# solislemuslab/BayesianNetworkRegression.jl

Measured on NVIDIA B200. Metric: gibbs_iters_per_sec_all_chains, higher is better.
Workload: dtype f64

## Files before the change

bayesiannetworkregression.jl_b200/csrc/bnr_linalg.cu:

```cuda
#include <cstdio>
#include <cstdlib>
#include <cstring>
#include <cuda.h>
#include "bnr_engine.cuh"
#include "bnr_kernels.h"

namespace bnr {

__device__ __forceinline__ void dmma884(double& c0, double& c1, double a, double b) {
  asm volatile("mma.sync.aligned.m8n8k4.row.col.f64.f64.f64.f64 {%0,%1}, {%2}, {%3}, {%0,%1};\n"
               : "+d"(c0), "+d"(c1) : "d"(a), "d"(b));
}
__device__ __forceinline__ double neg_bits(double x) {
  return __longlong_as_double(__double_as_longlong(x) ^ (long long)0x8000000000000000ull);
}
__device__ __forceinline__ void cp_async_commit() { asm volatile("cp.async.commit_group;\n" ::); }
template <int N>
__device__ __forceinline__ void cp_async_wait() { asm volatile("cp.async.wait_group %0;\n" ::"n"(N)); }
__device__ __forceinline__ void cp_async16(void* smem, const void* gmem) {
  const unsigned sa = (unsigned)__cvta_generic_to_shared(smem);
  asm volatile("cp.async.cg.shared.global [%0], [%1], 16;\n" ::"r"(sa), "l"(gmem));
}

__device__ __forceinline__ unsigned smem_u32(const void* p) { return (unsigned)__cvta_generic_to_shared(p); }
// ... 1191 lines not shown
#pragma unroll
        for (int h = 0; h < BW_NH; ++h)
#pragma unroll
          for (int q = 0; q < BW_CPW; ++q) bJ[h * BW_COLS + warp * BW_CPW + q] = xn[h][q];
      }
      __syncwarp();
      named_bar_sync(1, 256);
    }
    for (int id = tid; id < nown * PB; id += 256) {
      const int I = r + BWC_K * (id / PB);
      if (I < T) out[(size_t)c * out_stride + (size_t)I * PB + id % PB] = xo[id];
    }
  }
  cluster_sync_all();
}

__global__ void k_copy_sym(const double* __restrict__ G, size_t chain_stride, int np, double* __restrict__ out) {
  const int c = blockIdx.y, j = blockIdx.x;
  const double* Gc = G + (size_t)c * chain_stride;
  double* o = out + (size_t)c * np * np;
  for (int i = threadIdx.x; i < np; i += blockDim.x) {
    const double v = (i >= j) ? Gc[(size_t)j * np + i] : Gc[(size_t)i * np + j];
    o[(size_t)j * np + i] = v;
  }
}

constexpr int XM_BM = 128, XM_BN = 64, XM_BK = 16, XM_STAGES = 3;
constexpr int XM_LDM = 132, XM_LDK = 20;
constexpr int XM_A_DBL = (XM_BK * XM_LDM > XM_BM * XM_LDK) ? XM_BK * XM_LDM : XM_BM * XM_LDK;
constexpr int XM_STAGE_DBL = XM_A_DBL + XM_BN * XM_LDK;
constexpr size_t XMMA_SMEM = sizeof(double) * XM_STAGES * XM_STAGE_DBL;

__device__ __forceinline__ void cp_async16_zfill(void* smem, const void* gmem, bool valid) {
  const unsigned sa = (unsigned)__cvta_generic_to_shared(smem);
  const int sz = valid ? 16 : 0;
  asm volatile("cp.async.cg.shared.global [%0], [%1], 16, %2;\n" ::"r"(sa), "l"(gmem), "r"(sz));
}

template <int TRANS>
__global__ void __launch_bounds__(256) k_xmma(const double* __restrict__ X, int np, int M, int K, int N,
                                              const double* __restrict__ in, int ldin, double* __restrict__ out,
                                              int ldout, int k_per_split) {
  extern __shared__ __align__(16) double sm[];
  const int tid = threadIdx.x, lane = tid & 31, warp = tid >> 5;
  const int lk = lane & 3, lr = lane >> 2, wm = warp & 3, wn = warp >> 2;
  const int m0 = blockIdx.x * XM_BM, n0 = blockIdx.y * XM_BN;
  const int kbeg = blockIdx.z * k_per_split;
  const int kend = min(K, kbeg + k_per_split);
  const int nsteps = (kend - kbeg + XM_BK - 1) / XM_BK;
  double* o = out + (size_t)blockIdx.z * N * ldout;

  auto load_stage = [&](int step) {
    double* As = sm + (size_t)(step % XM_STAGES) * XM_STAGE_DBL;
    double* Vs = As + XM_A_DBL;
    const int k0 = kbeg + step * XM_BK;
    if (TRANS == 0) {
#pragma unroll
      for (int r = 0; r < 4; ++r) {
        const int id = tid + 256 * r, kk = id >> 6, mm = (id & 63) * 2;
        cp_async16_zfill(As + kk * XM_LDM + mm, X + (size_t)(k0 + kk) * np + m0 + mm, m0 + mm < M);
      }
    } else {
#pragma unroll
      for (int r = 0; r < 4; ++r) {
        const int id = tid + 256 * r, mm = id >> 3, kk = (id & 7) * 2;
        const bool ok = m0 + mm < M;
        cp_async16_zfill(As + mm * XM_LDK + kk, X + (size_t)(ok ? m0 + mm : 0) * np + k0 + kk, ok);
      }
    }
#pragma unroll
    for (int r = 0; r < 2; ++r) {
      const int id = tid + 256 * r, nn = id >> 3, kk = (id & 7) * 2;
      const bool ok = n0 + nn < N;
      cp_async16_zfill(Vs + nn * XM_LDK + kk, in + (size_t)(ok ? n0 + nn : 0) * ldin + k0 + kk, ok);
    }
  };

  double acc[4][4][2];
#pragma unroll
  for (int a = 0; a < 4; ++a)
#pragma unroll
    for (int b = 0; b < 4; ++b) acc[a][b][0] = acc[a][b][1] = 0.0;
  int nfv = (N - n0 - wn * 32 + 7) >> 3;
  nfv = nfv < 0 ? 0 : (nfv > 4 ? 4 : nfv);

  for (int s = 0; s < XM_STAGES - 1; ++s) {
    if (s < nsteps) load_stage(s);
    cp_async_commit();
  }
  for (int step = 0; step < nsteps; ++step) {
    cp_async_wait<XM_STAGES - 2>();
    __syncthreads();
    if (step + XM_STAGES - 1 < nsteps) load_stage(step + XM_STAGES - 1);
    cp_async_commit();
    const double* As = sm + (size_t)(step % XM_STAGES) * XM_STAGE_DBL;
    const double* Vs = As + XM_A_DBL;
    if (nfv == 0) continue;
#pragma unroll
    for (int k4 = 0; k4 < XM_BK / 4; ++k4) {
      const int kr = k4 * 4 + lk;
      double af[4], bf[4];
#pragma unroll
      for (int mf = 0; mf < 4; ++mf)
        af[mf] = (TRANS == 0) ? As[kr * XM_LDM + wm * 32 + mf * 8 + lr] : As[(wm * 32 + mf * 8 + lr) * XM_LDK + kr];
#pragma unroll
      for (int nf = 0; nf < 4; ++nf) bf[nf] = (nf < nfv) ? Vs[(wn * 32 + nf * 8 + lr) * XM_LDK + kr] : 0.0;
#pragma unroll
      for (int nf = 0; nf < 4; ++nf) {
        if (nf < nfv) {
#pragma unroll
          for (int mf = 0; mf < 4; ++mf) dmma884(acc[mf][nf][0], acc[mf][nf][1], af[mf], bf[nf]);
        }
      }
    }
  }
  cp_async_wait<0>();
#pragma unroll
  for (int mf = 0; mf < 4; ++mf) {
    const int mm = m0 + wm * 32 + mf * 8 + lr;
#pragma unroll
    for (int nf = 0; nf < 4; ++nf) {
      const int nn = n0 + wn * 32 + nf * 8 + 2 * lk;
      if (mm < M) {
        if (nn < N) o[(size_t)nn * ldout + mm] = acc[mf][nf][0];
        if (nn + 1 < N) o[(size_t)(nn + 1) * ldout + mm] = acc[mf][nf][1];
      }
    }
  }
}

__global__ void k_splitk_reduce(const double* __restrict__ ws, double* __restrict__ out, size_t count, int splits) {
  const size_t i = (size_t)blockIdx.x * blockDim.x + threadIdx.x;
  if (i >= count) return;
  double s = 0.0;
  for (int z = 0; z < splits; ++z) s += ws[(size_t)z * count + i];
  out[i] = s;
}

static int x_times_splits(const Dims& d, int trans) {
  const int M = trans ? d.qp : d.np, K = trans ? d.np : d.qp;
  const int tiles = ((M + XM_BM - 1) / XM_BM) * ((d.C_total + XM_BN - 1) / XM_BN);
  int ks = (2 * 148 + tiles - 1) / tiles;
  const int kmax = K / (4 * XM_BK) > 0 ? K / (4 * XM_BK) : 1;
  if (ks > kmax) ks = kmax;
  if (ks > 64) ks = 64;
  if (ks < 1) ks = 1;
  return ks;
}

size_t x_times_workspace_doubles(const Dims& d) {
  const int a = x_times_splits(d, 0), b = x_times_splits(d, 1);
  const size_t wa = (size_t)a * d.C_total * d.np, wb = (size_t)b * d.C_total * d.qp;
  return wa > wb ? wa : wb;
}

void launch_x_times(const Engine& e, int trans, const double* in, double* out, double* ws, cudaStream_t s) {
  const Dims& d = e.d;
  const int M = trans ? d.qp : d.np, K = trans ? d.np : d.qp, N = d.C;
  const int ldin = trans ? d.np : d.qp, ldout = trans ? d.qp : d.np;
  const int ks = x_times_splits(d, trans);
  const int kper = ((K + ks - 1) / ks + XM_BK - 1) / XM_BK * XM_BK;
  dim3 grid((M + XM_BM - 1) / XM_BM, (N + XM_BN - 1) / XM_BN, ks);
  double* dst = ks == 1 ? out : ws;
  ++g_launches;
  if (trans) k_xmma<1><<<grid, 256, XMMA_SMEM, s>>>(e.X, d.np, M, K, N, in, ldin, dst, ldout, kper);
  else k_xmma<0><<<grid, 256, XMMA_SMEM, s>>>(e.X, d.np, M, K, N, in, ldin, dst, ldout, kper);
  if (ks > 1) {
    const size_t count = (size_t)N * ldout;
    ++g_launches; k_splitk_reduce<<<(unsigned)((count + 255) / 256), 256, 0, s>>>(ws, out, count, ks);
  }
}

__global__ void k_gram_i8(const __grid_constant__ CUtensorMap tmA, const __grid_constant__ CUtensorMap tmB,
                          const double* __restrict__ rscale, double* __restrict__ G, int np, int nvalid, int nkb);
extern const size_t GI_SMEM_BYTES;

void linalg_setup() {
  cudaFuncSetAttribute(k_xmma<0>, cudaFuncAttributeMaxDynamicSharedMemorySize, (int)XMMA_SMEM);
  cudaFuncSetAttribute(k_xmma<1>, cudaFuncAttributeMaxDynamicSharedMemorySize, (int)XMMA_SMEM);
  cudaFuncSetAttribute(k_gram_syrk, cudaFuncAttributeMaxDynamicSharedMemorySize, (int)SYRK_SMEM);
  cudaFuncSetAttribute(k_gram_i8, cudaFuncAttributeMaxDynamicSharedMemorySize, (int)GI_SMEM_BYTES);
  cudaFuncSetAttribute(k_chol_update, cudaFuncAttributeMaxDynamicSharedMemorySize, (int)SYRK_SMEM);
  cudaFuncSetAttribute(k_trsm_dmma, cudaFuncAttributeMaxDynamicSharedMemorySize, (int)SYRK_SMEM);
  cudaFuncSetAttribute(k_potf2_inv, cudaFuncAttributeMaxDynamicSharedMemorySize, (int)POTF2_SMEM);
  cudaFuncSetAttribute(k_bwd_stream, cudaFuncAttributeMaxDynamicSharedMemorySize, 227 * 1024);
  cudaFuncSetAttribute(k_bwd_cluster, cudaFuncAttributeMaxDynamicSharedMemorySize, 227 * 1024);
  cudaFuncSetAttribute(k_small_tile<1, 4>, cudaFuncAttributeMaxDynamicSharedMemorySize, (int)small_tile_smem(32));
  cudaFuncSetAttribute(k_small_tile<2, 4>, cudaFuncAttributeMaxDynamicSharedMemorySize, (int)small_tile_smem(32));
  cudaFuncSetAttribute(k_small_tile<1, 2>, cudaFuncAttributeMaxDynamicSharedMemorySize, (int)small_tile_smem(16));
  cudaFuncSetAttribute(k_small_tile<2, 2>, cudaFuncAttributeMaxDynamicSharedMemorySize, (int)small_tile_smem(16));
  cudaFuncSetAttribute(k_small_tile<1, 8>, cudaFuncAttributeMaxDynamicSharedMemorySize, (int)small_tile_smem(64));
  cudaFuncSetAttribute(k_small_tile<2, 8>, cudaFuncAttributeMaxDynamicSharedMemorySize, (int)small_tile_smem(64));
}

typedef CUresult (*TmapEncodeFn)(CUtensorMap*, CUtensorMapDataType, cuuint32_t, void*, const cuuint64_t*, const cuuint64_t*,
                                 const cuuint32_t*, const cuuint32_t*, CUtensorMapInterleave, CUtensorMapSwizzle,
                                 CUtensorMapL2promotion, CUtensorMapFloatOOBfill);
static TmapEncodeFn g_tmap_encode = nullptr;
bool tmap_setup() {
  if (g_tmap_encode) return true;
  void* fn = nullptr;
  cudaDriverEntryPointQueryResult qr;
  if (cudaGetDriverEntryPoint("cuTensorMapEncodeTiled", &fn, cudaEnableDefault, &qr) != cudaSuccess ||
      qr != cudaDriverEntryPointSuccess || !fn)
    return false;
  g_tmap_encode = (TmapEncodeFn)fn;
  return true;
}
static CUresult encode_map(CUtensorMap* m, const double* base, uint64_t rows, uint64_t krows, uint64_t ld, uint32_t box_rows,
                           uint32_t box_k) {
  memset(m, 0, sizeof(*m));
  const cuuint64_t dims[2] = {rows, krows};
  const cuuint64_t strides[1] = {ld * sizeof(double)};
  const cuuint32_t box[2] = {box_rows, box_k};
  const cuuint32_t estr[2] = {1, 1};
  if (!tmap_setup()) return CUDA_ERROR_NOT_SUPPORTED;
  return g_tmap_encode(m, CU_TENSOR_MAP_DATA_TYPE_FLOAT64, 2, const_cast<double*>(base), dims, strides, box, estr,
                       CU_TENSOR_MAP_INTERLEAVE_NONE, CU_TENSOR_MAP_SWIZZLE_NONE, CU_TENSOR_MAP_L2_PROMOTION_L2_256B,
                       CU_TENSOR_MAP_FLOAT_OOB_FILL_NONE);
}
static CUtensorMap make_map(const double* base, uint64_t rows, uint64_t krows, uint64_t ld, uint32_t box_rows,
                            uint32_t box_k = SY_BK) {
  CUtensorMap m;
  const CUresult r = encode_map(&m, base, rows, krows, ld, box_rows, box_k);
  if (r != CUDA_SUCCESS) {
    fprintf(stderr, "[bnr] cuTensorMapEncodeTiled failed (%d) for a %llu x %llu operand, box %u x %d\n", (int)r,
            (unsigned long long)rows, (unsigned long long)krows, box_rows, (int)box_k);
    abort();
  }
  return m;
}
bool tmaps_check(const Engine& e) {
  const Dims& d = e.d;
  const uint64_t N = d.gdim, C = d.C, T = d.gdim / SY_BT;
  CUtensorMap m;
  bool ok = true;
  if (d.gmode != 2) ok = ok && encode_map(&m, e.X, d.np, d.qp, d.np, SY_LDS, SY_BK) == CUDA_SUCCESS;
  for (uint32_t box : {(uint32_t)SY_LDS, (uint32_t)(SY_BT / 2 + 4), (uint32_t)(SY_BT / 4 + 4)})
    ok = ok && encode_map(&m, e.G, N, N * C, N, box, SY_BK) == CUDA_SUCCESS;
  ok = ok && encode_map(&m, e.Linv, SY_BT, SY_BT * T * C, SY_BT, SY_LDS, SY_BK) == CUDA_SUCCESS;
  ok = ok && encode_map(&m, e.G, N, N * C, N, SY_BT, BW_COLS) == CUDA_SUCCESS;
  ok = ok && encode_map(&m, e.Linv, SY_BT, SY_BT * T * C, SY_BT, SY_BT, BW_COLS) == CUDA_SUCCESS;
  return ok;
}

int syrk_splits(const Dims& d, int C) {
  const int T = d.np / SY_BT, tiles = T * (T + 1) / 2, nk = d.qp / SY_BK;
  if (const char* ov = getenv("BNR_SYRK_SPLITS")) {
    int s = atoi(ov);
    if (s > nk / 8) s = nk / 8;
    return s < 1 ? 1 : (s > SYRK_MAX_SPLITS ? SYRK_MAX_SPLITS : s);
  }
  if (tiles * C >= 148) return 1;
  int s = (4 * 148 + tiles * C - 1) / (tiles * C);
  if (s > nk / 24) s = nk / 24;
  if (s > SYRK_MAX_SPLITS) s = SYRK_MAX_SPLITS;
  return s < 1 ? 1 : s;
}

#ifndef BNR_GI_BK
#define BNR_GI_BK 64
#endif
#ifndef BNR_GI_STAGES
#define BNR_GI_STAGES 2
#endif
constexpr int GI_S = 7;
constexpr int GI_BM = 128, GI_BN = 64;
constexpr int GI_BK = BNR_GI_BK;
constexpr int GI_STAGES = BNR_GI_STAGES;
constexpr int GI_A_PLANE = GI_BM * GI_BK, GI_B_PLANE = GI_BN * GI_BK;
constexpr int GI_STAGE_BYTES = GI_S * (GI_A_PLANE + GI_B_PLANE);
constexpr size_t GI_SMEM = (size_t)GI_STAGES * GI_STAGE_BYTES + 1024 + 256;
const size_t GI_SMEM_BYTES = GI_SMEM;
constexpr int GI_THREADS = 192;
static_assert(GI_BK == 32 || GI_BK == 64 || GI_BK == 128, "k-block = swizzle width");
static_assert(GI_S * GI_BN <= 512, "accumulators exceed tensor memory");

__device__ __forceinline__ unsigned long long gi_desc(unsigned saddr) {
  constexpr unsigned long long layout = GI_BK == 128 ? 2ull : (GI_BK == 64 ? 4ull : 6ull);
  return (unsigned long long)((saddr & 0x3FFFF) >> 4) | (1ull << 16) | ((unsigned long long)((GI_BK * 8) >> 4) << 32) |
         (1ull << 46) | (layout << 61);
}
__host__ __device__ constexpr unsigned gi_idesc(int n) {
  return (2u << 4) | (1u << 7) | (1u << 10) | ((unsigned)(n >> 3) << 17) | ((unsigned)(GI_BM >> 4) << 24);
}

__device__ __forceinline__ void tma_load_3d(void* smem_dst, const CUtensorMap* tm, int x, int y, int z, unsigned long long* bar) {
  asm volatile("cp.async.bulk.tensor.3d.shared::cluster.global.tile.mbarrier::complete_tx::bytes [%0], [%1, {%2, %3, %4}], [%5];\n" ::"r"(
                   smem_u32(smem_dst)), "l"((unsigned long long)tm), "r"(x), "r"(y), "r"(z), "r"(smem_u32(bar)) : "memory");
}
__device__ __forceinline__ void umma_i8(unsigned tmem_d, unsigned long long adesc, unsigned long long bdesc, unsigned idesc,
                                        bool acc) {
  asm volatile("{\n.reg .pred p;\nsetp.ne.b32 p, %4, 0;\ntcgen05.mma.cta_group::1.kind::i8 [%0], %1, %2, %3, p;\n}\n" ::"r"(tmem_d),
               "l"(adesc), "l"(bdesc), "r"(idesc), "r"((int)acc));
}
__device__ __forceinline__ void umma_commit(unsigned long long* bar) {
  asm volatile("tcgen05.commit.cta_group::1.mbarrier::arrive::one.shared::cluster.b64 [%0];\n" ::"r"(smem_u32(bar)) : "memory");
}
__device__ __forceinline__ void tmem_ld8(unsigned taddr, int (&r)[8]) {
  asm volatile("tcgen05.ld.sync.aligned.32x32b.x8.b32 {%0,%1,%2,%3,%4,%5,%6,%7}, [%8];\n"
               : "=r"(r[0]), "=r"(r[1]), "=r"(r[2]), "=r"(r[3]), "=r"(r[4]), "=r"(r[5]), "=r"(r[6]), "=r"(r[7]) : "r"(taddr));
}

__global__ void __launch_bounds__(256) k_gram_slice(const double* __restrict__ X, const double* __restrict__ S, int np,
                                                    int q, int qp, signed char* __restrict__ planes,
                                                    double* __restrict__ rscale) {
  __shared__ unsigned buf[GI_S][32][33];
  __shared__ double red[8][32];
  const int c = blockIdx.y, r0 = blockIdx.x * 32, lane = threadIdx.x & 31, warp = threadIdx.x >> 5;
  const int row = r0 + lane;
  const double* Sc = S + (size_t)c * qp;
  double m = 0.0;
  for (int k0 = warp; k0 < q; k0 += 8 * 32) {
    const int kl = k0 + 8 * lane;
    const double sq = kl < q ? sqrt(Sc[kl]) : 0.0;
    const int nk = (q - k0 + 7) / 8 < 32 ? (q - k0 + 7) / 8 : 32;
    for (int j = 0; j < nk; ++j) m = fmax(m, fabs(X[row + (size_t)np * (k0 + 8 * j)] * __shfl_sync(0xffffffffu, sq, j)));
  }
  red[warp][lane] = m;
  __syncthreads();
  m = 0.0;
#pragma unroll
  for (int w = 0; w < 8; ++w) m = fmax(m, red[w][lane]);
  int p = 0;
  if (m > 0.0) {
    p = 54 - ilogb(m);
    if (ldexp(m, p) > 126.0 * 0x1p48) --p;
  }
  if (warp == 0) rscale[(size_t)c * np + row] = ldexp(1.0, -p);
  const int p1 = p > 1000 ? 1000 : p;
  const double sc1 = ldexp(1.0, p1), sc2 = ldexp(1.0, p - p1);
  signed char* out = planes + (size_t)c * GI_S * np * qp;
  for (int k0 = 0; k0 < qp; k0 += 128) {
    const int kl = k0 + warp * 16 + (lane & 15);
    const double sq = kl < q ? sqrt(Sc[kl]) : 0.0;
#pragma unroll
    for (int g = 0; g < 4; ++g) {
      const int kw = warp * 4 + g;
      unsigned w[GI_S] = {0, 0, 0, 0, 0, 0, 0};
#pragma unroll
      for (int b = 0; b < 4; ++b) {
        const int k = k0 + kw * 4 + b;
        const double sqk = __shfl_sync(0xffffffffu, sq, g * 4 + b);
        if (k < q) {
          const long long M = __double2ll_rn(X[row + (size_t)np * k] * sqk * sc1 * sc2) + 0x808080808080ll;
          const unsigned lo = (unsigned)M ^ 0x80808080u, hi = (unsigned)(M >> 32) ^ 0x8080u;
#pragma unroll
          for (int i = 0; i < 4; ++i) w[GI_S - 1 - i] |= ((lo >> (8 * i)) & 255u) << (8 * b);
#pragma unroll
          for (int i = 0; i < 3; ++i) w[2 - i] |= ((hi >> (8 * i)) & 255u) << (8 * b);
        }
      }
#pragma unroll
      for (int s = 0; s < GI_S; ++s) buf[s][lane][kw] = w[s];
    }
    __syncthreads();
    for (int id = threadIdx.x; id < GI_S * 32 * 32; id += 256) {
      const int s = id >> 10, rr = (id >> 5) & 31, kw = id & 31;
      const int k = k0 + kw * 4;
      if (k < qp) *reinterpret_cast<unsigned*>(out + ((size_t)s * np + r0 + rr) * qp + k) = buf[s][rr][kw];
    }
    __syncthreads();
  }
}

__global__ void __launch_bounds__(GI_THREADS, 1)
k_gram_i8(const __grid_constant__ CUtensorMap tmA, const __grid_constant__ CUtensorMap tmB,
          const double* __restrict__ rscale, double* __restrict__ G, int np, int nvalid, int nkb) {
  extern __shared__ __align__(1024) unsigned char gsm_raw[];
  unsigned char* gsm = reinterpret_cast<unsigned char*>(((size_t)gsm_raw + 1023) & ~(size_t)1023);
  unsigned long long* full = reinterpret_cast<unsigned long long*>(gsm + (size_t)GI_STAGES * GI_STAGE_BYTES);
  unsigned long long* empty = full + GI_STAGES;
  unsigned long long* accf = empty + GI_STAGES;
  unsigned* tmem_slot = reinterpret_cast<unsigned*>(accf + 1);
  const int tid = threadIdx.x, lane = tid & 31, warp = tid >> 5;
  const int c = blockIdx.y;
  int ib = 0;
  while (2 * (ib + 1) * (ib + 2) / 2 <= (int)blockIdx.x) ++ib;
  const int jb = (int)blockIdx.x - ib * (ib + 1);
  const int i0 = ib * GI_BM, j0 = jb * GI_BN;
  const bool diag_block = (j0 / GI_BM) == ib;
  int rows_st = GI_BM;
  if (!diag_block) {
    int nfv = (nvalid - i0 + 7) / 8;
    if (nfv <= 0) return;
    rows_st = (nfv < 4 ? 4 : nfv) * 8;
  }
  if (tid == 0) {
    for (int s = 0; s < GI_STAGES; ++s) { mbar_init(&full[s], 1); mbar_init(&empty[s], 1); }
    mbar_init(accf, 1);
    asm volatile("fence.mbarrier_init.release.cluster;\n" ::: "memory");
  }
  if (warp == 0) {
    asm volatile("tcgen05.alloc.cta_group::1.sync.aligned.shared::cta.b32 [%0], 512;\n" ::"r"(smem_u32(tmem_slot)));
    asm volatile("tcgen05.relinquish_alloc_permit.cta_group::1.sync.aligned;\n");
  }
  asm volatile("tcgen05.fence::before_thread_sync;\n" ::: "memory");
  __syncthreads();
  asm volatile("tcgen05.fence::after_thread_sync;\n" ::: "memory");
  const unsigned tmem = *tmem_slot;

  if (warp == 4 && lane == 0) {
#if defined(GI_LAB_MMA_ONLY)
    for (int kb = 0; kb < GI_STAGES && kb < nkb; ++kb) {
#else
    for (int kb = 0; kb < nkb; ++kb) {
#endif
      const int st = kb % GI_STAGES;
      mbar_wait(&empty[st], ((kb / GI_STAGES) & 1) ^ 1);
      unsigned char* sa = gsm + (size_t)st * GI_STAGE_BYTES;
      mbar_expect_tx(&full[st], GI_STAGE_BYTES);
      tma_load_3d(sa, &tmA, kb * GI_BK, i0, c * GI_S, &full[st]);
      tma_load_3d(sa + GI_S * GI_A_PLANE, &tmB, kb * GI_BK, j0, c * GI_S, &full[st]);
    }
  } else if (warp == 5 && lane == 0) {
    for (int kb = 0; kb < nkb; ++kb) {
      const int st = kb % GI_STAGES;
#if defined(GI_LAB_MMA_ONLY)
      if (kb < GI_STAGES) mbar_wait(&full[st], 0);
#else
      mbar_wait(&full[st], (kb / GI_STAGES) & 1);
#endif
      asm volatile("tcgen05.fence::after_thread_sync;\n" ::: "memory");
#if defined(GI_LAB_LOADS_ONLY)
      umma_commit(&empty[st]);
      continue;
#endif
      const unsigned sa = smem_u32(gsm + (size_t)st * GI_STAGE_BYTES), sb = sa + GI_S * GI_A_PLANE;
#pragma unroll
      for (int kk = 0; kk < GI_BK / 32; ++kk) {
#pragma unroll
        for (int s = 0; s < GI_S; ++s) {
          const unsigned long long ad = gi_desc(sa + s * GI_A_PLANE + kk * 32);
#pragma unroll
          for (int t0 = 0; t0 < GI_S - s; t0 += 4) {
            const int nt = GI_S - s - t0 < 4 ? GI_S - s - t0 : 4;
            umma_i8(tmem + (unsigned)((s + t0) * GI_BN), ad, gi_desc(sb + t0 * GI_B_PLANE + kk * 32), gi_idesc(nt * GI_BN),
                    kb > 0 || kk > 0 || s > 0);
          }
        }
      }
      umma_commit(&empty[st]);
    }
    umma_commit(accf);
  } else if (warp < 4) {
    mbar_wait(accf, 0);
    asm volatile("tcgen05.fence::after_thread_sync;\n" ::: "memory");
    const int r = warp * 32 + lane, i = i0 + r;
    const double ri = rscale[(size_t)c * np + i] * 0x1p96;
    double* Gc = G + (size_t)c * np * np;
    const unsigned trow = tmem + ((unsigned)(warp * 32) << 16);
    for (int j8 = 0; j8 < GI_BN; j8 += 8) {
      int acc[GI_S][8];
#pragma unroll
      for (int g = 0; g < GI_S; ++g) tmem_ld8(trow + (unsigned)(g * GI_BN + j8), acc[g]);
      asm volatile("tcgen05.wait::ld.sync.aligned;\n" ::: "memory");
#pragma unroll
      for (int jj = 0; jj < 8; ++jj) {
        const int j = j0 + j8 + jj;
        double v = (double)acc[GI_S - 1][jj];
#pragma unroll
        for (int g = GI_S - 2; g >= 0; --g) v = (double)acc[g][jj] + v * 0x1p-8;
        v = v * ri * rscale[(size_t)c * np + j];
        if (i == j) v += 1.0;
        if (r < rows_st && (i >> 3) >= (j >> 3)) Gc[(size_t)j * np + i] = v;
      }
    }
  }
  asm volatile("tcgen05.fence::before_thread_sync;\n" ::: "memory");
  __syncthreads();
  if (warp == 0) {
    asm volatile("tcgen05.fence::after_thread_sync;\n" ::: "memory");
    asm volatile("tcgen05.dealloc.cta_group::1.sync.aligned.b32 %0, 512;\n" ::"r"(tmem));
  }
}

bool gram_i8_selected(const Dims& d) { return d.gmode == 1 && d.qp >= GRAM_I8_QP_MIN && d.qp <= GRAM_I8_QP_MAX; }

size_t gram_i8_plane_bytes(const Dims& d) { return (size_t)GI_S * d.np * d.qp; }

static CUresult encode_planes_map(CUtensorMap* m, const signed char* planes, const Dims& d, int C, uint32_t box_rows) {
  memset(m, 0, sizeof(*m));
  const cuuint64_t dims[3] = {(cuuint64_t)d.qp, (cuuint64_t)d.np, (cuuint64_t)GI_S * C};
  const cuuint64_t strides[2] = {(cuuint64_t)d.qp, (cuuint64_t)d.qp * d.np};
  const cuuint32_t box[3] = {(cuuint32_t)GI_BK, box_rows, (cuuint32_t)GI_S};
  const cuuint32_t estr[3] = {1, 1, 1};
  const CUtensorMapSwizzle sw = GI_BK == 128 ? CU_TENSOR_MAP_SWIZZLE_128B
                                             : (GI_BK == 64 ? CU_TENSOR_MAP_SWIZZLE_64B : CU_TENSOR_MAP_SWIZZLE_32B);
  if (!tmap_setup()) return CUDA_ERROR_NOT_SUPPORTED;
  return g_tmap_encode(m, CU_TENSOR_MAP_DATA_TYPE_UINT8, 3, const_cast<signed char*>(planes), dims, strides, box, estr,
                       CU_TENSOR_MAP_INTERLEAVE_NONE, sw, CU_TENSOR_MAP_L2_PROMOTION_L2_256B, CU_TENSOR_MAP_FLOAT_OOB_FILL_NONE);
}

static void launch_gram_i8_products(const Engine& e, cudaStream_t s) {
  const Dims& d = e.d;
  CUtensorMap tmA, tmB;
  if (encode_planes_map(&tmA, e.gram_planes, d, d.C, GI_BM) != CUDA_SUCCESS ||
      encode_planes_map(&tmB, e.gram_planes, d, d.C, GI_BN) != CUDA_SUCCESS) {
    fprintf(stderr, "[bnr] cuTensorMapEncodeTiled failed for the Gram digit planes (%d x %d)\n", d.np, d.qp);
    abort();
  }
  const int T = d.np / GI_BM;
  ++g_launches; k_gram_i8<<<dim3(T * (T + 1), d.C), GI_THREADS, GI_SMEM, s>>>(tmA, tmB, e.gram_rscale, e.G, d.np, d.n,
                                                                             (d.qp + GI_BK - 1) / GI_BK);
}

static void launch_gram_i8(const Engine& e, cudaStream_t s) {
  const Dims& d = e.d;
  ++g_launches; k_gram_slice<<<dim3(d.np / 32, d.C), 256, 0, s>>>(e.X, e.S, d.np, d.q, d.qp, e.gram_planes, e.gram_rscale);
  launch_gram_i8_products(e, s);
}

void launch_syrk_G(const Engine& e, cudaStream_t s) {
  const Dims& d = e.d;
  if (gram_i8_selected(d)) {
    launch_gram_i8(e, s);
    if (e.aux.G_copy) {
      dim3 g2(d.np, d.C);
      ++g_launches; k_copy_sym<<<g2, 256, 0, s>>>(e.G, (size_t)d.np * d.np, d.np, e.aux.G_copy);
    }
    return;
  }
  const int T = d.np / SY_BT;
  const int nk = d.qp / SY_BK;
  const int ns = e.syrk_ws ? e.syrk_ws_cap + 1 : 1;
  const int nk_split = (nk + ns - 1) / ns;
#if defined(SYRK_LAB_ONLY_DIAG)
  dim3 grid(d.C, ns, T);
#elif defined(SYRK_LAB_ONLY_OFFDIAG)
  dim3 grid(d.C, ns, T * (T - 1) / 2);
#else
  dim3 grid(d.C, ns, T * (T + 1) / 2);
#endif
  const size_t gs = (size_t)d.np * d.np;
  const CUtensorMap tmX = make_map(e.X, d.np, d.qp, d.np, SY_LDS);
  ++g_launches; k_gram_syrk<<<grid, SY_THREADS, SYRK_SMEM, s>>>(tmX, e.S, (size_t)d.qp, e.G, gs, d.np, d.n, nk, 1.0,
                                                            nk_split, e.syrk_ws, e.syrk_ws_cap);
  if (ns > 1) {
    dim3 g2(T * (T + 1) / 2 * 8, d.C);
    ++g_launches; k_syrk_splitk_reduce<<<g2, 256, 0, s>>>(e.G, gs, d.np, e.syrk_ws, e.syrk_ws_cap, ns - 1);
  }
  if (e.aux.G_copy) {
    dim3 g2(d.np, d.C);
    ++g_launches; k_copy_sym<<<g2, 256, 0, s>>>(e.G, gs, d.np, e.aux.G_copy);
  }
}

void launch_xtx(const Dims& d, const double* XT, const double* ones, double* XtX, cudaStream_t s) {
  const int T = d.qp / SY_BT;
  dim3 grid(1, 1, T * (T + 1) / 2);
  const CUtensorMap tmXT = make_map(XT, d.qp, d.np, d.qp, SY_LDS);
  ++g_launches; k_gram_syrk<<<grid, SY_THREADS, SYRK_SMEM, s>>>(tmXT, ones, 0, XtX, 0, d.qp, d.q, d.np / SY_BK, 0.0,
                                                            d.np / SY_BK, nullptr, 0);
}

__global__ void __launch_bounds__(256) k_build_P(Engine e) {
  const Dims& d = e.d;
  if (blockIdx.x < blockIdx.y) return;
  const int c = blockIdx.z, N = d.qp;
  const int i = blockIdx.x * 32 + threadIdx.x;
  const double it2 = 1.0 / e.tau2[c];
  double* Gc = e.G + (size_t)c * N * N;
#pragma unroll
  for (int jj = 0; jj < 4; ++jj) {
    const int j = blockIdx.y * 32 + threadIdx.y * 4 + jj;
    if (i < j) continue;
    double v;
    if (i < d.q) {
      v = e.XtX[(size_t)j * N + i] * it2;
      if (i == j) v = (e.XtX[(size_t)j * N + i] + 1.0 / e.S[(size_t)c * d.qp + j]) * it2;
    } else {
      v = (i == j) ? 1.0 : 0.0;
    }
    Gc[(size_t)j * N + i] = v;
  }
}

void launch_build_P(const Engine& e, cudaStream_t s) {
  const Dims& d = e.d;
  dim3 grid(d.qp / 32, d.qp / 32, d.C), block(32, 8);
  ++g_launches; k_build_P<<<grid, block, 0, s>>>(e);
  if (e.aux.G_copy) {
    dim3 g2(d.qp, d.C);
    ++g_launches; k_copy_sym<<<g2, 256, 0, s>>>(e.G, (size_t)d.qp * d.qp, d.qp, e.aux.G_copy);
  }
}

void launch_cholesky(const Engine& e, double* rhs, const ForkJoin& fj, cudaStream_t s) {
  const Dims& d = e.d;
  const int N = d.gdim;
  const int m = d.gmode == 2 ? d.q : d.n;
  const size_t cs = (size_t)N * N;
  const int T = N / PB;
  const size_t ls = (size_t)T * PB * PB;
  static const bool serial = getenv("BNR_CHOL_SERIAL") != nullptr;
  static const int forced = getenv("BNR_CHOL_SCHEDULE") ? atoi(getenv("BNR_CHOL_SCHEDULE")) : 0;
  const bool latency = forced ? forced == 2 : (long long)d.C_total * (T - 1) <= 128;
  ++g_launches; k_augment<<<d.C, 256, 0, s>>>(e.G, cs, N, m, rhs, d.gmode == 2 ? d.qp : d.np, d.gmode == 2 ? e.S : nullptr, e.tau2);
  const CUtensorMap mG = make_map(e.G, N, (uint64_t)N * d.C, N, SY_LDS);
  const CUtensorMap mG2 = make_map(e.G, N, (uint64_t)N * d.C, N, SY_BT / 2 + 4);
  const CUtensorMap mG4 = make_map(e.G, N, (uint64_t)N * d.C, N, SY_BT / 4 + 4);
  const CUtensorMap mL = make_map(e.Linv, PB, (uint64_t)PB * T * d.C, PB, SY_LDS);
  auto mI = [&](int ns) -> const CUtensorMap& { return ns == 4 ? mG4 : (ns == 2 ? mG2 : mG); };

  if (!latency) {
    const bool can_fork = !serial && fj.side != nullptr;
    static const bool a_lo = getenv("BNR_CHOL_A_SIDE_LO") != nullptr;
    cudaStream_t sideA = (!a_lo && fj.side_hi) ? fj.side_hi : fj.side;
    for (int J = 0; J < T; ++J) {
      const bool fork = can_fork && J > 0 && J + 1 < T;
      if (J > 0) {
        const int nk = J * PB / SY_BK;
        if (fork) {
          cudaEventRecord(fj.fork, s);
          cudaStreamWaitEvent(sideA, fj.fork, 0);
          dim3 g2(d.C, T - J - 1);
          ++g_launches; k_chol_update<<<g2, SY_THREADS, SYRK_SMEM, sideA>>>(mG, mG, 0, e.G, cs, N, m + 1, nk, J, J + 1, 1);
          cudaEventRecord(fj.join, sideA);
          dim3 g1(d.C, 1);
          ++g_launches; k_chol_update<<<g1, SY_THREADS, SYRK_SMEM, s>>>(mG, mG, 0, e.G, cs, N, m + 1, nk, J, J, 1);
        } else {
          dim3 g2(d.C, T - J);
          ++g_launches; k_chol_update<<<g2, SY_THREADS, SYRK_SMEM, s>>>(mG, mG, 0, e.G, cs, N, m + 1, nk, J, J, 1);
        }
      }
      ++g_launches; k_potf2_inv<<<d.C, 256, POTF2_SMEM, s>>>(e.G, cs, N, J, e.Linv, T, e.status, 0);
      if (fork) cudaStreamWaitEvent(s, fj.join, 0);
      if (J + 1 < T) {
        dim3 g1(d.C, T - J - 1);
        ++g_launches; k_trsm_dmma<<<g1, SY_THREADS, SYRK_SMEM, s>>>(mL, mG, e.G, cs, N, m + 1, J, J + 1, 1);
      }
    }
    return;
  }

  const bool fork = !serial && fj.side_hi != nullptr && fj.pool != nullptr && fj.npool >= 4 * T;
  cudaStream_t side = fork ? fj.side_hi : s;
  cudaEvent_t* evP = fj.pool;
  cudaEvent_t* evT = fj.pool + T;
  cudaEvent_t* evL = fj.pool + 2 * T;
  cudaEvent_t* evE = fj.pool + 3 * T;
  auto strips = [&](int tiles) {
    static const int fs = getenv("BNR_STRIPS") ? atoi(getenv("BNR_STRIPS")) : 0;
    if (fs == 1 || fs == 2 || fs == 4) return fs;
    const int ctas = d.C_total * tiles;
    return ctas * 4 <= 148 ? 4 : (ctas * 2 <= 148 ? 2 : 1);
  };
  static const bool small_tiles = getenv("BNR_NO_SMALL_TILES") == nullptr;
  auto launch_trsm = [&](int J, int ib_first, int rows, int ns, cudaStream_t st) {
    dim3 g(d.C, rows * ns);
    const double* Lj = e.Linv + (size_t)J * PB * PB;
    ++g_launches;
    if (small_tiles && ns == 8)
      k_small_tile<2, 2><<<g, 256, small_tile_smem(16), st>>>(e.G, cs, N, J, ib_first, 8, Lj, ls, PB, J * PB, 0);
    else if (small_tiles && ns == 4)
      k_small_tile<2, 4><<<g, 256, small_tile_smem(32), st>>>(e.G, cs, N, J, ib_first, 4, Lj, ls, PB, J * PB, 0);
    else if (small_tiles && ns == 2)
      k_small_tile<2, 8><<<g, 256, small_tile_smem(64), st>>>(e.G, cs, N, J, ib_first, 2, Lj, ls, PB, J * PB, 0);
    else
      k_trsm_dmma<<<g, SY_THREADS, SYRK_SMEM, st>>>(mL, mI(ns), e.G, cs, N, m + 1, J, ib_first, ns);
  };
  static const int ud_knob = getenv("BNR_CHOL_UD") ? atoi(getenv("BNR_CHOL_UD")) : -1;
  const bool quiet = d.gmode == 2 || e.syrk_ws != nullptr;
  int ud = (small_tiles && quiet) ? (d.C_total * 8 <= 148 ? 8 : (d.C_total * 4 <= 148 ? 4 : 0)) : 0;
  if (ud_knob == 0 || ud_knob == 4 || ud_knob == 8) ud = small_tiles ? ud_knob : 0;
  for (int J = 0; J < T; ++J) {
    const bool has_side = J + 2 < T;
    if (fork && J >= 2 && !ud) cudaStreamWaitEvent(s, evE[J - 2], 0);
    ++g_launches; k_potf2_inv<<<d.C, 256, POTF2_SMEM, s>>>(e.G, cs, N, J, e.Linv, T, e.status, (J > 0 && !ud) ? 1 : 0);
    if (fork && has_side) cudaEventRecord(evP[J], s);
    if (J + 1 < T) {
      if (fork && J >= 1 && J + 1 < T) cudaStreamWaitEvent(s, evL[J - 1], 0);
      const int ns1 = ud ? ud : strips(1);
      launch_trsm(J, J + 1, 1, ns1, s);
      if (fork && has_side) cudaEventRecord(evT[J], s);
      if (ud) {
        if (fork && J >= 1) cudaStreamWaitEvent(s, evE[J - 1], 0);
        dim3 gd(d.C, ud);
        const double* Lt = e.G + (size_t)J * PB * N + (size_t)(J + 1) * PB;
        ++g_launches;
        if (ud == 8) k_small_tile<1, 2><<<gd, 256, small_tile_smem(16), s>>>(e.G, cs, N, J + 1, J + 1, 8, Lt, cs, N, J * PB, 1);
        else k_small_tile<1, 4><<<gd, 256, small_tile_smem(32), s>>>(e.G, cs, N, J + 1, J + 1, 4, Lt, cs, N, J * PB, 1);
      }
    }
    if (has_side) {
      const int rows = T - J - 2;
      if (fork) cudaStreamWaitEvent(side, evP[J], 0);
      const int ns2 = strips(rows);
      dim3 g2(d.C, rows * ns2);
      launch_trsm(J, J + 2, rows, ns2, side);
      if (fork) cudaStreamWaitEvent(side, evT[J], 0);
      ++g_launches;
      if (small_tiles && ns2 == 4)
        k_small_tile<1, 4><<<g2, 256, small_tile_smem(32), side>>>(e.G, cs, N, J + 1, J + 2, 4, e.G + (size_t)J * PB * N + (size_t)(J + 1) * PB, cs, N, J * PB, 0);
      else if (small_tiles && ns2 == 2)
        k_small_tile<1, 8><<<g2, 256, small_tile_smem(64), side>>>(e.G, cs, N, J + 1, J + 2, 2, e.G + (size_t)J * PB * N + (size_t)(J + 1) * PB, cs, N, J * PB, 0);
      else
        k_chol_update<<<g2, SY_THREADS, SYRK_SMEM, side>>>(mG, mI(ns2), J * PB, e.G, cs, N, m + 1, PB / SY_BK, J + 1, J + 2, ns2);
      if (fork) cudaEventRecord(evL[J], side);
      ++g_launches; k_chol_update<<<g2, SY_THREADS, SYRK_SMEM, side>>>(mG, mI(ns2), 0, e.G, cs, N, m + 1, (J + 1) * PB / SY_BK,
                                                                   J + 2, J + 2, ns2);
      if (fork) cudaEventRecord(evE[J], side);
    }
  }
}

void launch_chol_solve(const Engine& e, double* out, const double* addz, cudaStream_t s) {
  const Dims& d = e.d;
  const int N = d.gdim;
  const int m = d.gmode == 2 ? d.q : d.n;
  const int stride = d.gmode == 2 ? d.qp : d.np;
  const CUtensorMap tmG = make_map(e.G, N, (uint64_t)N * d.C, N, PB, BW_COLS);
  const CUtensorMap tmL = make_map(e.Linv, PB, (uint64_t)PB * (N / PB) * d.C, PB, PB, BW_COLS);
  if (N <= BWD_STREAM_MAX_DIM) {
    ++g_launches; k_bwd_stream<<<d.C, BW_THREADS, bwd_smem(N), s>>>(tmG, tmL, e.G, (size_t)N * N, N, m, out, stride, addz,
                                                                 stride, bwd_stages(N));
    return;
  }
  cudaLaunchConfig_t cfg = {};
  cudaLaunchAttribute attr[1];
  attr[0].id = cudaLaunchAttributeClusterDimension;
  attr[0].val.clusterDim.x = BWC_K; attr[0].val.clusterDim.y = 1; attr[0].val.clusterDim.z = 1;
  cfg.gridDim = dim3(d.C * BWC_K);
  cfg.blockDim = dim3(BW_THREADS);
  cfg.dynamicSmemBytes = bwc_smem(N);
  cfg.stream = s;
  cfg.attrs = attr;
  cfg.numAttrs = 1;
  ++g_launches;
  cudaLaunchKernelEx(&cfg, k_bwd_cluster, tmG, tmL, (const double*)e.G, (size_t)N * N, N, m, out, stride, addz, stride,
                     bwc_stages(N));
}

int bwd_cluster_capacity(int N) {
  if (N <= BWD_STREAM_MAX_DIM) return 1;
  cudaLaunchConfig_t cfg = {};
  cudaLaunchAttribute attr[1];
  attr[0].id = cudaLaunchAttributeClusterDimension;
  attr[0].val.clusterDim.x = BWC_K; attr[0].val.clusterDim.y = 1; attr[0].val.clusterDim.z = 1;
  cfg.gridDim = dim3(BWC_K);
  cfg.blockDim = dim3(BW_THREADS);
  cfg.dynamicSmemBytes = bwc_smem(N);
  cfg.attrs = attr;
  cfg.numAttrs = 1;
  int n = 0;
  if (cudaOccupancyMaxActiveClusters(&n, k_bwd_cluster, &cfg) != cudaSuccess) return -1;
  return n;
}

int chol_max_dim() { return CHOL_MAX_DIM; }
int bwd_stream_max_dim() { return BWD_STREAM_MAX_DIM; }

}
```

Before: 10760.

## Restructure Gram digit-slicing kernel to share X loads across chains

Rewrites k_gram_slice so each block handles 16 rows and 4 chains. X is loaded once into registers and reused across chains, and the sqrt(S) values are staged in padded shared memory instead of being broadcast by shuffle. Bytes are packed with __byte_perm and written as 16-byte vector stores straight to global memory, replacing the shared-memory transpose buffer. It also adds compile-time lab switches that disable stores or digit computation for experiments. The cost is higher register pressure and fewer blocks in the grid.

```diff
diff --git a/bayesiannetworkregression.jl_b200/csrc/bnr_linalg.cu b/bayesiannetworkregression.jl_b200/csrc/bnr_linalg.cu
--- a/bayesiannetworkregression.jl_b200/csrc/bnr_linalg.cu
+++ b/bayesiannetworkregression.jl_b200/csrc/bnr_linalg.cu
@@ -1517,66 +1517,137 @@
                : "=r"(r[0]), "=r"(r[1]), "=r"(r[2]), "=r"(r[3]), "=r"(r[4]), "=r"(r[5]), "=r"(r[6]), "=r"(r[7]) : "r"(taddr));
 }
 
-__global__ void __launch_bounds__(256) k_gram_slice(const double* __restrict__ X, const double* __restrict__ S, int np,
-                                                    int q, int qp, signed char* __restrict__ planes,
-                                                    double* __restrict__ rscale) {
-  __shared__ unsigned buf[GI_S][32][33];
-  __shared__ double red[8][32];
-  const int c = blockIdx.y, r0 = blockIdx.x * 32, lane = threadIdx.x & 31, warp = threadIdx.x >> 5;
-  const int row = r0 + lane;
-  const double* Sc = S + (size_t)c * qp;
-  double m = 0.0;
-  for (int k0 = warp; k0 < q; k0 += 8 * 32) {
-    const int kl = k0 + 8 * lane;
-    const double sq = kl < q ? sqrt(Sc[kl]) : 0.0;
-    const int nk = (q - k0 + 7) / 8 < 32 ? (q - k0 + 7) / 8 : 32;
-    for (int j = 0; j < nk; ++j) m = fmax(m, fabs(X[row + (size_t)np * (k0 + 8 * j)] * __shfl_sync(0xffffffffu, sq, j)));
-  }
-  red[warp][lane] = m;
+constexpr int GS_ROWS = 16, GS_CB = 4, GS_THREADS = 256, GS_TK = 512;
+constexpr int GS_TKP = GS_TK + GS_TK / 8;
+__device__ __forceinline__ int gs_tidx(int kk) { return kk + 2 * (kk >> 4); }
+
+__device__ __forceinline__ void gs_roots(double (*sq)[GS_TKP], const double* __restrict__ S, int qp, int q, int ncb, int t0) {
+  for (int id = threadIdx.x; id < GS_CB * GS_TK; id += GS_THREADS) {
+    const int cb = id / GS_TK, kk = id % GS_TK, k = t0 + kk;
+    sq[cb][gs_tidx(kk)] = cb < ncb && k < q ? sqrt(S[(size_t)cb * qp + k]) : 0.0;
+  }
+}
+
+__device__ __forceinline__ void gs_load_x(double (&x)[16], const double* __restrict__ X, int np, int q, int row, int k0) {
+  const bool full = k0 + 16 <= q;
+#pragma unroll
+  for (int j = 0; j < 16; ++j) x[j] = full || k0 + j < q ? X[row + (size_t)np * (k0 + j)] : 0.0;
+}
+
+__global__ void __launch_bounds__(GS_THREADS, 2) k_gram_slice(const double* __restrict__ X, const double* __restrict__ S,
+                                                            int np, int q, int qp, int C, signed char* __restrict__ planes,
+                                                            double* __restrict__ rscale) {
+  __shared__ __align__(16) double sq[GS_CB][GS_TKP];
+  __shared__ double red[GS_THREADS / 32][GS_CB][GS_ROWS];
+  __shared__ double2 scl[GS_CB][GS_ROWS];
+  const int lane = threadIdx.x & 31, warp = threadIdx.x >> 5, rr = lane & 15, h = lane >> 4;
+  const int r0 = blockIdx.x * GS_ROWS, row = r0 + rr, c0 = blockIdx.y * GS_CB;
+  const int ncb = C - c0 < GS_CB ? C - c0 : GS_CB;
+  const double* Sb = S + (size_t)c0 * qp;
+  constexpr int NW = GS_THREADS / 32, BPW = GS_TK / 32 / NW;
+  double x[16];
+
+  double m[GS_CB];
+#pragma unroll
+  for (int cb = 0; cb < GS_CB; ++cb) m[cb] = 0.0;
+  for (int t0 = 0; t0 < q; t0 += GS_TK) {
+    __syncthreads();
+    gs_roots(sq, Sb, qp, q, ncb, t0);
+    __syncthreads();
+#pragma unroll
+    for (int i = 0; i < BPW; ++i) {
+      const int kk = 32 * (warp + NW * i) + 16 * h;
+      if (t0 + kk >= q) continue;
+      gs_load_x(x, X, np, q, row, t0 + kk);
+#pragma unroll
+      for (int cb = 0; cb < GS_CB; ++cb) {
+        if (cb >= ncb) break;
+#pragma unroll
+        for (int j = 0; j < 16; j += 2) {
+          const double2 s2 = *reinterpret_cast<const double2*>(&sq[cb][gs_tidx(kk + j)]);
+          m[cb] = fmax(m[cb], fabs(x[j] * s2.x));
+          m[cb] = fmax(m[cb], fabs(x[j + 1] * s2.y));
+        }
+      }
+    }
+  }
+#pragma unroll
+  for (int cb = 0; cb < GS_CB; ++cb) {
+    const double o = __shfl_xor_sync(0xffffffffu, m[cb], 16);
+    if (h == 0) red[warp][cb][rr] = fmax(m[cb], o);
+  }
   __syncthreads();
-  m = 0.0;
-#pragma unroll
-  for (int w = 0; w < 8; ++w) m = fmax(m, red[w][lane]);
-  int p = 0;
-  if (m > 0.0) {
-    p = 54 - ilogb(m);
-    if (ldexp(m, p) > 126.0 * 0x1p48) --p;
-  }
-  if (warp == 0) rscale[(size_t)c * np + row] = ldexp(1.0, -p);
-  const int p1 = p > 1000 ? 1000 : p;
-  const double sc1 = ldexp(1.0, p1), sc2 = ldexp(1.0, p - p1);
-  signed char* out = planes + (size_t)c * GI_S * np * qp;
-  for (int k0 = 0; k0 < qp; k0 += 128) {
-    const int kl = k0 + warp * 16 + (lane & 15);
-    const double sq = kl < q ? sqrt(Sc[kl]) : 0.0;
-#pragma unroll
-    for (int g = 0; g < 4; ++g) {
-      const int kw = warp * 4 + g;
-      unsigned w[GI_S] = {0, 0, 0, 0, 0, 0, 0};
-#pragma unroll
-      for (int b = 0; b < 4; ++b) {
-        const int k = k0 + kw * 4 + b;
-        const double sqk = __shfl_sync(0xffffffffu, sq, g * 4 + b);
-        if (k < q) {
-          const long long M = __double2ll_rn(X[row + (size_t)np * k] * sqk * sc1 * sc2) + 0x808080808080ll;
-          const unsigned lo = (unsigned)M ^ 0x80808080u, hi = (unsigned)(M >> 32) ^ 0x8080u;
-#pragma unroll
-          for (int i = 0; i < 4; ++i) w[GI_S - 1 - i] |= ((lo >> (8 * i)) & 255u) << (8 * b);
-#pragma unroll
-          for (int i = 0; i < 3; ++i) w[2 - i] |= ((hi >> (8 * i)) & 255u) << (8 * b);
-        }
-      }
-#pragma unroll
-      for (int s = 0; s < GI_S; ++s) buf[s][lane][kw] = w[s];
-    }
+  if (threadIdx.x < GS_CB * GS_ROWS) {
+    const int cb = threadIdx.x / GS_ROWS, i = threadIdx.x % GS_ROWS;
+    double mx = 0.0;
+#pragma unroll
+    for (int w = 0; w < NW; ++w) mx = fmax(mx, red[w][cb][i]);
+    int p = 0;
+    if (mx > 0.0) {
+      p = 54 - ilogb(mx);
+      if (ldexp(mx, p) > 126.0 * 0x1p48) --p;
+    }
+    if (cb < ncb) rscale[(size_t)(c0 + cb) * np + r0 + i] = ldexp(1.0, -p);
+    const int p1 = p > 1000 ? 1000 : p;
+    scl[cb][i] = make_double2(ldexp(1.0, p1), ldexp(1.0, p - p1));
+  }
+
+#if defined(GS_LAB_NO_STORES)
+  unsigned sink = 0;
+#endif
+  for (int t0 = 0; t0 < qp; t0 += GS_TK) {
     __syncthreads();
-    for (int id = threadIdx.x; id < GI_S * 32 * 32; id += 256) {
-      const int s = id >> 10, rr = (id >> 5) & 31, kw = id & 31;
-      const int k = k0 + kw * 4;
-      if (k < qp) *reinterpret_cast<unsigned*>(out + ((size_t)s * np + r0 + rr) * qp + k) = buf[s][rr][kw];
-    }
+    gs_roots(sq, Sb, qp, q, ncb, t0);
     __syncthreads();
-  }
+#pragma unroll 1
+    for (int i = 0; i < BPW; ++i) {
+      const int kk = 32 * (warp + NW * i) + 16 * h;
+      if (t0 + kk >= qp) continue;
+      gs_load_x(x, X, np, q, row, t0 + kk);
+#pragma unroll 1
+      for (int cb = 0; cb < ncb; ++cb) {
+        const double2 sc = scl[cb][rr];
+        uint4 w[GI_S];
+#pragma unroll
+        for (int g = 0; g < 4; ++g) {
+          unsigned lo[4], hi[4];
+#pragma unroll
+          for (int b = 0; b < 4; ++b) {
+            const int j = 4 * g + b;
+#if defined(GS_LAB_NO_DIGITS)
+            lo[b] = __double2loint(x[j]) + j; hi[b] = __double2hiint(x[j]) + cb;
+#else
+            const double sqk = sq[cb][gs_tidx(kk + j)];
+            const unsigned long long M = (unsigned long long)__double2ll_rn(x[j] * sqk * sc.x * sc.y) + 0x808080808080ull;
+            lo[b] = (unsigned)M; hi[b] = (unsigned)(M >> 32);
+#endif
+          }
+          const unsigned a0 = __byte_perm(lo[0], lo[1], 0x5140), a1 = __byte_perm(lo[0], lo[1], 0x7362);
+          const unsigned a2 = __byte_perm(lo[2], lo[3], 0x5140), a3 = __byte_perm(lo[2], lo[3], 0x7362);
+          const unsigned b0 = __byte_perm(hi[0], hi[1], 0x5140), b1 = __byte_perm(hi[0], hi[1], 0x7362);
+          const unsigned b2 = __byte_perm(hi[2], hi[3], 0x5140), b3 = __byte_perm(hi[2], hi[3], 0x7362);
+          const unsigned v[GI_S] = {__byte_perm(b1, b3, 0x5410), __byte_perm(b0, b2, 0x7632) ^ 0x80808080u,
+                                    __byte_perm(b0, b2, 0x5410) ^ 0x80808080u, __byte_perm(a1, a3, 0x7632) ^ 0x80808080u,
+                                    __byte_perm(a1, a3, 0x5410) ^ 0x80808080u, __byte_perm(a0, a2, 0x7632) ^ 0x80808080u,
+                                    __byte_perm(a0, a2, 0x5410) ^ 0x80808080u};
+#pragma unroll
+          for (int s = 0; s < GI_S; ++s) (&w[s].x)[g] = v[s];
+        }
+        signed char* out = planes + ((size_t)(c0 + cb) * GI_S * np + row) * qp + t0 + kk;
+#pragma unroll
+        for (int s = 0; s < GI_S; ++s) {
+#if defined(GS_LAB_NO_STORES)
+          sink ^= w[s].x ^ w[s].y ^ w[s].z ^ w[s].w;
+#else
+          *reinterpret_cast<uint4*>(out + (size_t)s * np * qp) = w[s];
+#endif
+        }
+      }
+    }
+  }
+#if defined(GS_LAB_NO_STORES)
+  if (sink == 0x9e3779b9u) planes[0] = 1;
+#endif
 }
 
 __global__ void __launch_bounds__(GI_THREADS, 1)
@@ -1720,9 +1791,14 @@
                                                                              (d.qp + GI_BK - 1) / GI_BK);
 }
 
+static void launch_gram_slice(const Engine& e, cudaStream_t s) {
+  const Dims& d = e.d;
+  ++g_launches; k_gram_slice<<<dim3(d.np / GS_ROWS, (d.C + GS_CB - 1) / GS_CB), GS_THREADS, 0, s>>>(
+      e.X, e.S, d.np, d.q, d.qp, d.C, e.gram_planes, e.gram_rscale);
+}
+
 static void launch_gram_i8(const Engine& e, cudaStream_t s) {
-  const Dims& d = e.d;
-  ++g_launches; k_gram_slice<<<dim3(d.np / 32, d.C), 256, 0, s>>>(e.X, e.S, d.np, d.q, d.qp, e.gram_planes, e.gram_rscale);
+  launch_gram_slice(e, s);
   launch_gram_i8_products(e, s);
 }
 
```

New measurement: 11870 (median of 6 runs). 10.2% higher.
